# twice154/ofa-for-super-resolution

Hardware: AMD Instinct MI355X
Metric: sr_training_images_per_sec_4x_64to256 (higher is better)
Workload: dtype bf16; 1 GPU; OFA-SR S4 supernet 4x progressive shrinking (elastic kernel {3,5,7}, e=6, d=4, pd=2), LR 64x64 -> HR 256x256, fwd+bwd+Adam, train-mode BN; kernel_transform_mode=1, compat_reference_indexing=True, parallelism=dp1, per_gpu_batch=16, global_batch=16, grad_allreduce_bytes=0, launch=eager

## Files before the change

### include/ofasr.h

```cpp
#ifndef OFASR_H
#define OFASR_H

#include <stddef.h>
#include <stdint.h>

#ifdef __cplusplus
extern "C" {
#endif

#define OFASR_VERSION 312

typedef enum {
    OFASR_OK = 0,
    OFASR_ERR_INVALID_ARG = -1,
    OFASR_ERR_UNSUPPORTED = -2,
    OFASR_ERR_WORKSPACE = -3,
    OFASR_ERR_LAUNCH = -4
} ofasr_status;

typedef enum { OFASR_F32 = 0, OFASR_F16 = 1, OFASR_BF16 = 2 } ofasr_dtype;

int ofasr_version(void);
const char* ofasr_last_error_string(void);
const char* ofasr_status_string(int status);
// ... 130 lines not shown
                              void* stream);

size_t ofasr_conv2d_workspace(int64_t Cin, int64_t Cout, int K, int dgrad);
int ofasr_conv2d_stat_units(int64_t N, int64_t Cin, int64_t Cout, int64_t H, int64_t W, int K);
int ofasr_conv2d_fwd_stat(const void* x, const float* w, void* y, int64_t N, int64_t Cin, int64_t Cout, int64_t H,
                          int64_t W, int K, int dtype, void* partial, int64_t units, void* workspace,
                          size_t workspace_bytes, void* stream);
int ofasr_bn_fwd_cp(const void* x, const void* residual, void* y, const void* partial, int64_t P, const float* gamma,
                    const float* beta, float* running_mean, float* running_var, double momentum, double eps, int training,
                    float* stats, int64_t N, int64_t C, int64_t HW, int act, int dtype, void* stream);
int ofasr_bn_finalize_cp(const void* partial, int64_t P, int64_t C, double count, const float* gamma, const float* beta,
                         float* running_mean, float* running_var, double momentum, double eps, int training, float* stats,
                         void* stream);
int ofasr_pixel_shuffle2_bn(const void* x, void* y, const float* stats, int64_t N, int64_t C, int64_t H, int64_t W,
                            int dtype, void* stream);
size_t ofasr_bn_bwd_ps2_workspace(int64_t N, int64_t C);
int ofasr_bn_bwd_ps2(const void* dout, const void* x, void* dx, const float* scale, const float* mean, const float* invstd,
                     float* dgamma, float* dbeta, int64_t N, int64_t C, int64_t H, int64_t W, int training, int dtype,
                     void* workspace, size_t workspace_bytes, void* stream);
size_t ofasr_conv2d_infer_operand_bytes(int64_t Cin, int64_t Cout, int K);
int ofasr_conv2d_infer_prepare(const float* w, const float* gamma, const float* beta, const float* running_mean,
                               const float* running_var, double eps, int64_t Cin, int64_t Cout, int K, int dtype,
                               void* operands, size_t operand_bytes, void* stream);
int ofasr_conv2d_infer_run(const void* x, void* y, int64_t N, int64_t Cin, int64_t Cout, int64_t H, int64_t W, int K,
                           int dtype, int act, const void* operands, size_t operand_bytes, void* stream);
int ofasr_conv2d_fwd(const void* x, const float* w, void* y, int64_t N, int64_t Cin, int64_t Cout, int64_t H, int64_t W,
                     int K, int dtype, void* workspace, size_t workspace_bytes, void* stream);
int ofasr_conv2d_dgrad(const void* dy, const float* w, void* dx, int64_t N, int64_t Cin, int64_t Cout, int64_t H,
                       int64_t W, int K, int dtype, void* workspace, size_t workspace_bytes, void* stream);
size_t ofasr_conv2d_wgrad_workspace(int64_t N, int64_t Cin, int64_t Cout, int64_t H, int64_t W, int K);
int ofasr_conv2d_wgrad(const void* dy, const void* x, float* dw, int64_t N, int64_t Cin, int64_t Cout, int64_t H,
                       int64_t W, int K, int dtype, void* workspace, size_t workspace_bytes, void* stream);

size_t ofasr_conv2d_f32_workspace(int64_t Cin, int64_t Cout, int K, int dgrad);
// ... 117 lines not shown
```

### ofa-for-super-resolution_amd/_C.py

```python
import ctypes
import os
import subprocess

import torch

_HERE = os.path.dirname(os.path.abspath(__file__))
LIB_PATH = os.environ.get("OFASR_LIB_PATH") or os.path.join(_HERE, "csrc", "libofasr_hip.so")

F32, F16, BF16 = 0, 1, 2
U8_HWC = 3

_lib = None

_c_i64 = ctypes.c_int64
_c_int = ctypes.c_int
_c_vp = ctypes.c_void_p
_c_sz = ctypes.c_size_t

SIGNATURES = {
    "ofasr_version": (_c_int, []),
    "ofasr_last_error_string": (ctypes.c_char_p, []),
    "ofasr_status_string": (ctypes.c_char_p, [_c_int]),
    "ofasr_pixel_shuffle": (_c_int, [_c_vp, _c_vp, _c_i64, _c_i64, _c_i64, _c_i64, _c_int, _c_int, _c_vp]),
    "ofasr_pixel_unshuffle": (_c_int, [_c_vp, _c_vp, _c_i64, _c_i64, _c_i64, _c_i64, _c_int, _c_int, _c_vp]),
# ... 21 lines not shown
                                  _c_vp]),
    "ofasr_bn_fwd": (_c_int, [_c_vp, _c_vp, _c_vp, _c_vp, _c_vp, _c_vp, _c_vp, ctypes.c_double, ctypes.c_double, _c_int,
                              _c_vp, _c_i64, _c_i64, _c_i64, _c_int, _c_int, _c_vp, _c_sz, _c_vp]),
    "ofasr_bn_act_bwd_workspace": (_c_sz, [_c_i64, _c_i64]),
    "ofasr_bn_act_bwd": (_c_int, [_c_vp, _c_vp, _c_vp, _c_vp, _c_vp, _c_vp, _c_vp, _c_vp, _c_vp, _c_vp, _c_vp,
                                  _c_i64, _c_i64, _c_i64, _c_int, _c_int, _c_int, _c_vp, _c_sz, _c_vp]),
    "ofasr_conv2d_workspace": (_c_sz, [_c_i64, _c_i64, _c_int, _c_int]),
    "ofasr_conv2d_stat_units": (_c_int, [_c_i64, _c_i64, _c_i64, _c_i64, _c_i64, _c_int]),
    "ofasr_conv2d_fwd_stat": (_c_int, [_c_vp, _c_vp, _c_vp, _c_i64, _c_i64, _c_i64, _c_i64, _c_i64, _c_int, _c_int, _c_vp,
                                       _c_i64, _c_vp, _c_sz, _c_vp]),
    "ofasr_bn_fwd_cp": (_c_int, [_c_vp, _c_vp, _c_vp, _c_vp, _c_i64, _c_vp, _c_vp, _c_vp, _c_vp, ctypes.c_double,
                                 ctypes.c_double, _c_int, _c_vp, _c_i64, _c_i64, _c_i64, _c_int, _c_int, _c_vp]),
    "ofasr_bn_finalize_cp": (_c_int, [_c_vp, _c_i64, _c_i64, ctypes.c_double, _c_vp, _c_vp, _c_vp, _c_vp, ctypes.c_double,
                                      ctypes.c_double, _c_int, _c_vp, _c_vp]),
    "ofasr_pixel_shuffle2_bn": (_c_int, [_c_vp, _c_vp, _c_vp, _c_i64, _c_i64, _c_i64, _c_i64, _c_int, _c_vp]),
    "ofasr_bn_bwd_ps2_workspace": (_c_sz, [_c_i64, _c_i64]),
    "ofasr_bn_bwd_ps2": (_c_int, [_c_vp, _c_vp, _c_vp, _c_vp, _c_vp, _c_vp, _c_vp, _c_vp, _c_i64, _c_i64, _c_i64, _c_i64, _c_int,
                                  _c_int, _c_vp, _c_sz, _c_vp]),
    "ofasr_conv2d_infer_operand_bytes": (_c_sz, [_c_i64, _c_i64, _c_int]),
    "ofasr_conv2d_infer_prepare": (_c_int, [_c_vp, _c_vp, _c_vp, _c_vp, _c_vp, ctypes.c_double, _c_i64, _c_i64, _c_int, _c_int,
                                            _c_vp, _c_sz, _c_vp]),
    "ofasr_conv2d_infer_run": (_c_int, [_c_vp, _c_vp, _c_i64, _c_i64, _c_i64, _c_i64, _c_i64, _c_int, _c_int, _c_int, _c_vp,
                                        _c_sz, _c_vp]),
    "ofasr_conv2d_fwd": (_c_int, [_c_vp, _c_vp, _c_vp, _c_i64, _c_i64, _c_i64, _c_i64, _c_i64, _c_int, _c_int, _c_vp,
                                  _c_sz, _c_vp]),
    "ofasr_conv2d_dgrad": (_c_int, [_c_vp, _c_vp, _c_vp, _c_i64, _c_i64, _c_i64, _c_i64, _c_i64, _c_int, _c_int, _c_vp,
                                    _c_sz, _c_vp]),
    "ofasr_conv2d_wgrad_workspace": (_c_sz, [_c_i64, _c_i64, _c_i64, _c_i64, _c_i64, _c_int]),
    "ofasr_conv2d_wgrad": (_c_int, [_c_vp, _c_vp, _c_vp, _c_i64, _c_i64, _c_i64, _c_i64, _c_i64, _c_int, _c_int, _c_vp,
                                    _c_sz, _c_vp]),
# ... 180 lines not shown
```

### ofa-for-super-resolution_amd/csrc/conv2d.hip

```cpp
#include "ofasr_common.h"

namespace ofasr {

typedef __attribute__((ext_vector_type(16))) float cv_f32x16;
typedef __attribute__((ext_vector_type(8))) __bf16 cv_bf16x8;
typedef __attribute__((ext_vector_type(8))) _Float16 cv_f16x8;
typedef __attribute__((ext_vector_type(8))) short cv_s16x8;

constexpr int CV_TW = 64;
constexpr int CV_SEG = 20;
constexpr int CV_RP = 4 * CV_SEG;
constexpr int CV_KC = 32;

template <typename T> struct CvMma;
template <> struct CvMma<bf16_t> {
    static __device__ __forceinline__ cv_f32x16 run(cv_s16x8 a, cv_s16x8 b, cv_f32x16 c) {
        return __builtin_amdgcn_mfma_f32_32x32x16_bf16(__builtin_bit_cast(cv_bf16x8, a), __builtin_bit_cast(cv_bf16x8, b),
                                                       c, 0, 0, 0);
    }
};
template <> struct CvMma<f16_t> {
    static __device__ __forceinline__ cv_f32x16 run(cv_s16x8 a, cv_s16x8 b, cv_f32x16 c) {
        return __builtin_amdgcn_mfma_f32_32x32x16_f16(__builtin_bit_cast(cv_f16x8, a), __builtin_bit_cast(cv_f16x8, b), c,
                                                      0, 0, 0);
    }
};

__device__ __forceinline__ int cv_pos(int r, int col) { return r * CV_RP + (col & 3) * CV_SEG + (col >> 2); }
__device__ __forceinline__ int cv_rec(int P, int j) { return P * 64 + ((j ^ ((P >> 2) & 3)) << 4); }

struct CvBn {
    float* ss;
    const float* gamma;
    const float* beta;
    const float* mean;
    const float* var;
    float eps;
};

template <typename T>
__global__ void __launch_bounds__(256) conv_prep_kernel(const float* __restrict__ w, T* __restrict__ wimg, int Cin,
                                                        int KS, int dgrad, int M, int Kdim, int nrb, long long total,
                                                        CvBn bn) {
    const long long idx = (long long)blockIdx.x * blockDim.x + threadIdx.x;
    if (bn.ss != nullptr && idx < M) {
        float sc = 1.f, sh = 0.f;
        if (bn.gamma != nullptr) {
            sc = bn.gamma[idx] * rsqrtf(bn.var[idx] + bn.eps);
            sh = bn.beta[idx] - bn.mean[idx] * sc;
        }
        bn.ss[idx] = sc;
        bn.ss[M + idx] = sh;
    }
    if (idx >= total) return;
    const int j = (int)(idx & 7), lane = (int)((idx >> 3) & 63);
    long long t = idx >> 9;
    const int rb = (int)(t % nrb);
    t /= nrb;
    const int tx = (int)(t % KS);
    t /= KS;
    const int s = (int)(t & 1);
    t >>= 1;
    const int ty = (int)(t % KS);
    const int kc = (int)(t / KS);
    const int m = rb * 32 + (lane & 31), kk = kc * CV_KC + 16 * s + 8 * (lane >> 5) + j;
    float v = 0.f;
    if (m < M && kk < Kdim) {
        const int taps = KS * KS, tap = ty * KS + tx;
        v = dgrad ? w[((long long)kk * Cin + m) * taps + (taps - 1 - tap)]
                  : w[((long long)m * Cin + kk) * taps + tap];
    }
    wimg[idx] = from_float<T>(v);
}

__device__ __forceinline__ void cv_lds_barrier() { asm volatile("s_waitcnt lgkmcnt(0)\n\ts_barrier" ::: "memory"); }

struct CvEpi {
    const float* ss;
    int act;
    float2* stat;
    int P;
};

template <typename T, int KS, int RB, int WM, int WP, bool ONEK>
__global__ void __launch_bounds__(64 * WM * WP, 2) conv_igemm_kernel(const T* __restrict__ x, const T* __restrict__ wimg,
                                                                     T* __restrict__ y, int Cx, int M, int H, int W,
                                                                     int tiles_x, int nkc, int nrb, CvEpi epi) {
// ... 211 lines not shown
    p.M = (int)(dgrad ? Cin : Cout);
    p.Kdim = (int)(dgrad ? Cout : Cin);
    p.ok = (K == 3 || K == 5) && p.M > 0 && p.Kdim > 0;
    p.cfg = p.M > 128 ? 0 : (p.M > 64 ? 1 : (p.M > 32 ? 2 : 3));
    if (p.cfg == 2 && N > 0 && N * cdiv(H, 8) * cdiv(W, CV_TW) < 512) p.cfg = 4;
    p.rows = p.cfg == 0 ? 256 : (p.cfg == 1 ? 128 : (p.cfg == 3 ? 32 : 64));
    p.th = p.cfg == 0 ? 2 : ((p.cfg == 1 || p.cfg == 4) ? 4 : 8);
    p.threads = 256;
    p.nslab = (int)cdiv(p.M, p.rows);
    p.nrb = p.nslab * (p.rows / 32);
    p.nkc = (int)cdiv(p.Kdim, CV_KC);
    p.img_bytes = (size_t)p.nkc * K * 2 * K * p.nrb * 1024;
    return p;
}

template <typename T>
static int launch_conv_prep(const char* name, const float* w, int64_t Cin, int64_t Cout, int K, int dgrad, void* ws, CvBn bn,
                            hipStream_t st) {
    const CvPlan p = cv_plan(Cin, Cout, K, dgrad);
    const long long total = (long long)(p.img_bytes / 2);
    OFASR_LAUNCH((conv_prep_kernel<T>), dim3((unsigned)cdiv(total, 256)), dim3(256), 0, st, w, (T*)ws, (int)Cin, K,
                       dgrad, p.M, p.Kdim, p.nrb, total, bn);
    return check_launch(name);
}

template <typename T>
static int launch_conv_run(const char* name, const void* x, const void* ws, void* y, int64_t N, int64_t Cin, int64_t Cout,
                           int64_t H, int64_t W, int K, int dgrad, CvEpi epi, hipStream_t st) {
    const CvPlan p = cv_plan(Cin, Cout, K, dgrad, N, H, W);
    const int tiles_x = (int)cdiv(W, CV_TW), tiles_y = (int)cdiv(H, p.th);
    dim3 grid((unsigned)(tiles_x * tiles_y), (unsigned)N, (unsigned)p.nslab);
    prof_note((double)sizeof(T) * (double)N * (double)H * (double)W * (double)(Cin + Cout),
              2.0 * (double)N * (double)H * (double)W * (double)Cin * (double)Cout * K * K);
#define OFASR_CV(KS, RB, WM, WP, ONEK)                                                                                  \
    OFASR_LAUNCH((conv_igemm_kernel<T, KS, RB, WM, WP, ONEK>), grid, dim3(64 * WM * WP), 0, st, (const T*)x,         \
                       (const T*)ws, (T*)y, p.Kdim, p.M, (int)H, (int)W, tiles_x, p.nkc, p.nrb, epi)
#define OFASR_CVK(KS, ONEK)                                                                                         \
// ... 5 lines not shown
        default: OFASR_CV(KS, 1, 1, 4, ONEK); break;                                                                \
    }
    const bool onek = p.Kdim <= 16;
    if (K == 5) {
        if (onek) { OFASR_CVK(5, true) } else { OFASR_CVK(5, false) }
    } else {
        if (onek) { OFASR_CVK(3, true) } else { OFASR_CVK(3, false) }
    }
#undef OFASR_CVK
#undef OFASR_CV
    return check_launch(name);
}

template <typename T>
static int launch_conv2d(const char* name, const void* x, const float* w, void* y, int64_t N, int64_t Cin, int64_t Cout,
                         int64_t H, int64_t W, int K, int dgrad, void* ws, hipStream_t st, StatOut so = StatOut{nullptr, 0}) {
    int rc = launch_conv_prep<T>(name, w, Cin, Cout, K, dgrad, ws, CvBn{}, st);
    if (rc) return rc;
    return launch_conv_run<T>(name, x, ws, y, N, Cin, Cout, H, W, K, dgrad, CvEpi{nullptr, 0, so.partial, so.P}, st);
}

typedef __attribute__((ext_vector_type(4))) short cv_s16x4;
typedef __attribute__((address_space(3))) cv_s16x4 cv_lds_s16x4;

struct CvWgParams {
    int Cin, Cout, H, W, tiles_x, tiles_y, ntiles, ksplit, ncislab, nz;
};

template <int WCI> __device__ __forceinline__ int cvw_xoff(int R, int chunk) {
    if constexpr (WCI == 2) return R * 128 + ((((chunk >> 2) ^ ((R >> 1) & 1))) << 6) + ((chunk & 3) << 4);
    else return R * 64 + (chunk << 4);
}

// ... 264 lines not shown
    return check_launch(name);
}

static int conv_stat_units(int64_t N, int64_t Cin, int64_t Cout, int64_t H, int64_t W, int K) {
    if (conv_thin_out_supported(Cout, Cin, K, W, OFASR_BF16, nullptr, nullptr))
        return conv_thin_out_units(N, Cout, Cin, H, W, OFASR_BF16);
    if (conv_thin_in_supported(Cin, Cout, K, W, OFASR_BF16, nullptr, nullptr))
        return conv_thin_in_units(N, Cin, Cout, H, W, OFASR_BF16);
    const CvPlan p = cv_plan(Cin, Cout, K, 0, N, H, W);
    const int wp = p.th / 2;
    return (int)(N * cdiv(W, CV_TW) * cdiv(H, p.th) * wp);
}

static int conv2d_entry(const char* name, const void* x, const float* w, void* y, int64_t N, int64_t Cin, int64_t Cout,
                        int64_t H, int64_t W, int K, int dtype, int dgrad, void* ws, size_t ws_bytes, void* stream,
                        StatOut so = StatOut{nullptr, 0}) {
    OFASR_REQUIRE(x && w && y, OFASR_ERR_INVALID_ARG, "%s: null pointer", name);
    OFASR_REQUIRE(N > 0 && Cin > 0 && Cout > 0 && H > 0 && W > 0, OFASR_ERR_INVALID_ARG, "%s: bad shape", name);
    OFASR_REQUIRE(dtype == OFASR_F16 || dtype == OFASR_BF16, OFASR_ERR_UNSUPPORTED,
                  "%s: 16-bit activations only (fp32 runs on the vendor library)", name);
    OFASR_REQUIRE(K == 3 || K == 5, OFASR_ERR_UNSUPPORTED, "%s: K=%d not in {3,5}", name, K);
    OFASR_REQUIRE(W % 8 == 0 && ((reinterpret_cast<uintptr_t>(x) | reinterpret_cast<uintptr_t>(y)) & 15) == 0,
                  OFASR_ERR_UNSUPPORTED, "%s: needs W %% 8 == 0 and 16-byte aligned tensors", name);
    OFASR_REQUIRE(N <= 65535 && H * W <= (1LL << 31), OFASR_ERR_UNSUPPORTED, "%s: too large", name);
    const CvPlan p = cv_plan(Cin, Cout, K, dgrad);
    OFASR_REQUIRE(ws && ws_bytes >= p.img_bytes, OFASR_ERR_WORKSPACE, "%s: workspace %zu B < required %zu B", name,
                  ws_bytes, p.img_bytes);
    hipStream_t st = as_stream(stream);
    {
        const int64_t Ct = dgrad ? Cin : Cout, Cw = dgrad ? Cout : Cin;
        if (conv_thin_out_supported(Ct, Cw, K, W, dtype, x, y)) {
            if (so.partial)
                OFASR_REQUIRE(!dgrad && so.P == conv_thin_out_units(N, Ct, Cw, H, W, dtype), OFASR_ERR_INVALID_ARG,
                              "%s: statistics unit count %d does not match the launch", name, so.P);
            return conv_thin_out(x, w, y, N, Ct, Cw, H, W, K, dtype, dgrad, so, stream);
        }
        if (conv_thin_in_supported(Cw, Ct, K, W, dtype, x, y)) {
            if (so.partial)
                OFASR_REQUIRE(!dgrad && so.P == conv_thin_in_units(N, Cw, Ct, H, W, dtype), OFASR_ERR_INVALID_ARG,
                              "%s: statistics unit count %d does not match the launch", name, so.P);
            return conv_thin_in(x, w, y, N, Cw, Ct, H, W, K, dtype, dgrad, so, stream);
        }
    }
    if (so.partial)
        OFASR_REQUIRE(!dgrad && so.P == conv_stat_units(N, Cin, Cout, H, W, K), OFASR_ERR_INVALID_ARG,
                      "%s: statistics unit count %d does not match the launch", name, so.P);
    if (dtype == OFASR_BF16) return launch_conv2d<bf16_t>(name, x, w, y, N, Cin, Cout, H, W, K, dgrad, ws, st, so);
    return launch_conv2d<f16_t>(name, x, w, y, N, Cin, Cout, H, W, K, dgrad, ws, st, so);
}

}

using namespace ofasr;

OFASR_EXPORT size_t ofasr_conv2d_workspace(int64_t Cin, int64_t Cout, int K, int dgrad) {
    if (Cin <= 0 || Cout <= 0 || !(K == 3 || K == 5)) return 0;
    return cv_plan(Cin, Cout, K, dgrad).img_bytes;
}

OFASR_EXPORT int ofasr_conv2d_fwd(const void* x, const float* w, void* y, int64_t N, int64_t Cin, int64_t Cout, int64_t H,
                                  int64_t W, int K, int dtype, void* workspace, size_t workspace_bytes, void* stream) {
    return conv2d_entry("ofasr_conv2d_fwd", x, w, y, N, Cin, Cout, H, W, K, dtype, 0, workspace, workspace_bytes, stream);
}
// ... 53 lines not shown
                                       int64_t W, int K, int dtype, void* partial, int64_t units, void* workspace,
                                       size_t workspace_bytes, void* stream) {
    OFASR_REQUIRE(partial != nullptr && units > 0 && units <= INT32_MAX, OFASR_ERR_INVALID_ARG,
                  "ofasr_conv2d_fwd_stat: null / empty statistics buffer");
    return conv2d_entry("ofasr_conv2d_fwd_stat", x, w, y, N, Cin, Cout, H, W, K, dtype, 0, workspace, workspace_bytes, stream,
                        StatOut{(float2*)partial, (int)units});
}

OFASR_EXPORT int ofasr_conv2d_dgrad(const void* dy, const float* w, void* dx, int64_t N, int64_t Cin, int64_t Cout,
                                    int64_t H, int64_t W, int K, int dtype, void* workspace, size_t workspace_bytes,
                                    void* stream) {
    return conv2d_entry("ofasr_conv2d_dgrad", dy, w, dx, N, Cin, Cout, H, W, K, dtype, 1, workspace, workspace_bytes,
                        stream);
}

OFASR_EXPORT size_t ofasr_conv2d_wgrad_workspace(int64_t N, int64_t Cin, int64_t Cout, int64_t H, int64_t W, int K) {
    if (N <= 0 || Cin <= 0 || Cout <= 0 || H <= 0 || W <= 0 || !(K == 3 || K == 5)) return 0;
    size_t need = cv_wg_plan(N, Cin, Cout, H, W, K).part_bytes;
    const int64_t Ct = Cin < Cout ? Cin : Cout, Cw = Cin < Cout ? Cout : Cin;
    if (conv_thin_wgrad_supported(Ct, Cw, K, H, W, OFASR_BF16, nullptr, nullptr)) {
        const size_t thin = conv_thin_wgrad_workspace(N, Ct, Cw, H, W, K, OFASR_BF16);
        need = thin > need ? thin : need;
    }
    return need;
}

OFASR_EXPORT int ofasr_conv2d_wgrad(const void* dy, const void* x, float* dw, int64_t N, int64_t Cin, int64_t Cout,
                                    int64_t H, int64_t W, int K, int dtype, void* workspace, size_t workspace_bytes,
                                    void* stream) {
    const char* name = "ofasr_conv2d_wgrad";
// ... 21 lines not shown
```

### ofa-for-super-resolution_amd/csrc/pixel_shuffle.hip

```cpp
#include "ofasr_common.h"

namespace ofasr {

template <typename U, bool SHUFFLE>
__global__ void __launch_bounds__(256) ps_generic_kernel(const U* __restrict__ x, U* __restrict__ y,
                                                         int64_t total, int C, int H, int W, int r) {
    const int Ho = H * r, Wo = W * r;
    for (int64_t idx = (int64_t)blockIdx.x * blockDim.x + threadIdx.x; idx < total;
         idx += (int64_t)gridDim.x * blockDim.x) {
        int wo = (int)(idx % Wo);
        int64_t t = idx / Wo;
        int ho = (int)(t % Ho);
        t /= Ho;
        int c = (int)(t % C);
        int64_t n = t / C;
        int h = ho / r, i = ho % r, w = wo / r, j = wo % r;
        int64_t lr = (((n * C + c) * r * r + i * r + j) * H + h) * (int64_t)W + w;
        if (SHUFFLE) y[idx] = x[lr];
        else y[lr] = x[idx];
    }
}

template <int ES> struct Interleave;
template <> struct Interleave<4> {
// ... 86 lines not shown
#pragma unroll
        for (int j = 0; j < 4; ++j) {
            const float mu = mean[c0 + j], sc = scale[c0 + j];
            v[j] = ps_bn8<T>(v[j], mu, sc, fmaf(mu, sc, shift[c0 + j]));
        }
        uint4 lo, hi;
        Interleave<2>::zip(v[0], v[1], lo, hi);
        dst[hr0] = lo;
        dst[hr0 + 1] = hi;
        Interleave<2>::zip(v[2], v[3], lo, hi);
        dst[hr0 + 2 * Wq] = lo;
        dst[hr0 + 2 * Wq + 1] = hi;
    }
}

template <bool SHUFFLE>
static int launch(const void* x, void* y, int64_t N, int64_t C, int64_t H, int64_t W, int r, int es,
                  hipStream_t st) {
    const char* name = SHUFFLE ? "ofasr_pixel_shuffle" : "ofasr_pixel_unshuffle";
    OFASR_REQUIRE(x && y, OFASR_ERR_INVALID_ARG, "%s: null pointer", name);
    OFASR_REQUIRE(N >= 0 && C >= 0 && H >= 0 && W >= 0 && r >= 1, OFASR_ERR_INVALID_ARG,
                  "%s: bad shape N=%lld C=%lld H=%lld W=%lld r=%d", name, (long long)N, (long long)C,
                  (long long)H, (long long)W, r);
    OFASR_REQUIRE(es == 1 || es == 2 || es == 4 || es == 8, OFASR_ERR_UNSUPPORTED,
                  "%s: elem_size %d not in {1,2,4,8}", name, es);
    OFASR_REQUIRE(C <= INT32_MAX && H * r <= INT32_MAX && W * r <= INT32_MAX, OFASR_ERR_UNSUPPORTED,
                  "%s: dimension too large", name);
    const int64_t total = N * C * r * r * H * W;
    if (total == 0) return OFASR_OK;
    prof_note(2.0 * (double)total * es, 0.0);
// ... 53 lines not shown
    const float *mean = stats, *scale = stats + 2 * Cin, *shift = stats + 3 * Cin;
    const int Wq = (int)(W / 8);
    const int64_t items = N * C * H * Wq;
    const int64_t blocks = cdiv(items, 256);
    const int grid = (int)(blocks < 65536 ? blocks : 65536);
    hipStream_t st = as_stream(stream);
    prof_note(2.0 * 2.0 * (double)N * (double)Cin * (double)H * (double)W, 0.0);
    if (dtype == OFASR_BF16)
        OFASR_LAUNCH((ps_r2_bn_kernel<bf16_t>), dim3(grid), dim3(256), 0, st, (const uint4*)x, (uint4*)y, mean, scale, shift, items,
                     (int)C, (int)H, Wq);
    else
        OFASR_LAUNCH((ps_r2_bn_kernel<f16_t>), dim3(grid), dim3(256), 0, st, (const uint4*)x, (uint4*)y, mean, scale, shift, items,
                     (int)C, (int)H, Wq);
    return check_launch(name);
}
```

### ofa-for-super-resolution_amd/ops.py

```python
import collections
import ctypes
import os
import weakref

import torch
from torch.autograd import Function
from torch.autograd.function import once_differentiable

from . import _C

_DT = {torch.float32: _C.F32, torch.float16: _C.F16, torch.bfloat16: _C.BF16}


def _dt(t):
    try:
        return _DT[t.dtype]
    except KeyError:
        raise _C.OfasrError("unsupported activation dtype %s (f32/f16/bf16 only)" % t.dtype)


def _gpu(*ts):
    for t in ts:
        if t is None:
            continue
# ... 634 lines not shown
        if ctx.needs_input_grad[1]:
            dw = torch.zeros_like(w)
            wst, wsp, wsn = _ws(L.ofasr_pwconv_wgrad_workspace(N, Cin, cout, H * W), x.device)
            with _timed("pwconv_wgrad_%dx%d" % (cout, Cin), (x.numel() + dy.numel()) * x.element_size() + 4 * Cin * cout,
                        2 * Cin * cout * N * H * W):
                _C.check(L.ofasr_pwconv_wgrad(_p(dy), _p(x), _p(dw), ldw, N, Cin, cout, H * W, _dt(x), wsp, wsn,
                                              _stream()), "pwconv_wgrad")
        return dx, dw, None


def pwconv(x, w_full, cout):
    return PWConvFn.apply(x, w_full, cout)


ACT_NONE, ACT_RELU6 = 0, 1


class BNActFn(Function):

    @staticmethod
    def forward(ctx, x, weight, bias, running_mean, running_var, training, momentum, eps, act, residual):
        _gpu(x, weight, bias, running_mean, running_var, residual)
        x = x.contiguous()
        N, C, H, W = x.shape
        HW = H * W
        L = _C.lib()
        dev = x.device
        w = _f32_param(weight)
        b = _f32_param(bias)
        stats = torch.empty((4, C), dtype=torch.float32, device=dev)
# ... 47 lines not shown
    return dx, dgamma, dbeta, dres


class BNActCPFn(Function):

    @staticmethod
    def forward(ctx, x, partial, weight, bias, running_mean, running_var, momentum, eps, act):
        _gpu(x, weight, bias, running_mean, running_var)
        N, C, H, W = x.shape
        L = _C.lib()
        w, b = _f32_param(weight), _f32_param(bias)
        stats = torch.empty((4, C), dtype=torch.float32, device=x.device)
        units = partial.shape[1]
        if act == ACT_PIXEL_SHUFFLE2:
            y = torch.empty((N, C // 4, 2 * H, 2 * W), dtype=x.dtype, device=x.device)
            _C.check(L.ofasr_bn_finalize_cp(_p(partial), units, C, float(N * H * W), _p(w), _p(b), _p(running_mean),
                                            _p(running_var), float(momentum), float(eps), 1, _p(stats), _stream()),
                     "bn_finalize_cp")
            with _timed("bn_pixel_shuffle", 2 * x.numel() * x.element_size()):
                _C.check(L.ofasr_pixel_shuffle2_bn(_p(x), _p(y), _p(stats), N, C // 4, H, W, _dt(x), _stream()),
                         "pixel_shuffle2_bn")
        else:
            y = torch.empty_like(x)
            with _timed("bn_fwd_cp", 2 * x.numel() * x.element_size()):
                _C.check(L.ofasr_bn_fwd_cp(_p(x), None, _p(y), _p(partial), units, _p(w), _p(b), _p(running_mean),
                                           _p(running_var), float(momentum), float(eps), 1, _p(stats), N, C, H * W, int(act),
                                           _dt(x), _stream()), "bn_fwd_cp")
        ctx.save_for_backward(x, stats)
        ctx.meta = (True, ACT_NONE if act == ACT_PIXEL_SHUFFLE2 else act, False, tuple(weight.shape))
        ctx.shuffled = act == ACT_PIXEL_SHUFFLE2
        return y

    @staticmethod
    @once_differentiable
    def backward(ctx, dy):
        x, stats = ctx.saved_tensors
# ... 654 lines not shown
            return dx, None
        return dx, dw


class Conv2dFn(Function):

    @staticmethod
    def forward(ctx, x, weight, dgrad_hip=True):
        x = _al16(x.contiguous())
        N, Cin, H, W = x.shape
        Cout, _, K, _ = weight.shape
        ctx.dgrad_hip = dgrad_hip
        L = _C.lib()
        y = torch.empty((N, Cout, H, W), dtype=x.dtype, device=x.device)
        wst, wsp, wsn = _ws(L.ofasr_conv2d_workspace(Cin, Cout, K, 0), x.device)
        with _timed("conv2d_fwd_%dto%d_k%d" % (Cin, Cout, K), (x.numel() + y.numel()) * x.element_size(),
                    2 * N * H * W * Cin * Cout * K * K):
            _C.check(L.ofasr_conv2d_fwd(_p(x), _p(weight), _p(y), N, Cin, Cout, H, W, K, _dt(x), wsp, wsn, _stream()),
                     "conv2d_fwd")
        ctx.save_for_backward(x, weight)
        return y

    @staticmethod
    @once_differentiable
    def backward(ctx, dy):
        return _conv2d_backward(ctx, dy)


class Conv2dStatFn(Function):

    @staticmethod
    def forward(ctx, x, weight):
        x = _al16(x.contiguous())
        N, Cin, H, W = x.shape
        Cout, _, K, _ = weight.shape
        ctx.dgrad_hip = True
        L = _C.lib()
        y = torch.empty((N, Cout, H, W), dtype=x.dtype, device=x.device)
        units = L.ofasr_conv2d_stat_units(N, Cin, Cout, H, W, K)
        partial = torch.empty((Cout, units, 2), dtype=torch.float32, device=x.device)
        wst, wsp, wsn = _ws(L.ofasr_conv2d_workspace(Cin, Cout, K, 0), x.device)
        with _timed("conv2d_fwd_%dto%d_k%d" % (Cin, Cout, K), (x.numel() + y.numel()) * x.element_size(),
                    2 * N * H * W * Cin * Cout * K * K):
            _C.check(L.ofasr_conv2d_fwd_stat(_p(x), _p(weight), _p(y), N, Cin, Cout, H, W, K, _dt(x), _p(partial), units,
                                             wsp, wsn, _stream()), "conv2d_fwd_stat")
        ctx.save_for_backward(x, weight)
        ctx.mark_non_differentiable(partial)
        return y, partial

    @staticmethod
    @once_differentiable
    def backward(ctx, dy, _dpartial):
        return _conv2d_backward(ctx, dy)[:2]


def _conv2d_backward(ctx, dy):
    x, weight = ctx.saved_tensors
    N, Cin, H, W = x.shape
    Cout, _, K, _ = weight.shape
    dy = _al16(dy.contiguous())
    L = _C.lib()
    dx = dw = None
    if not ctx.dgrad_hip:
        w16 = weight.to(x.dtype)
        dx, dw, _ = torch.ops.aten.convolution_backward(dy, x, w16, None, [1, 1], [K // 2, K // 2], [1, 1], False,
                                                        [0, 0], 1, [ctx.needs_input_grad[0],
                                                                    ctx.needs_input_grad[1], False])
        return dx, (dw.float() if dw is not None else None), None
    cur = torch.cuda.current_stream(x.device)
    side = _side_stream(x.device) if (ctx.needs_input_grad[0] and ctx.needs_input_grad[1] and SIDE_STREAM) else None
    defer = False
    if ctx.needs_input_grad[1] and side is None and CONV_DEFER_WGRAD and H * W >= CONV_DEFER_MIN_HW \
# ... 12 lines not shown
            with torch.cuda.stream(side if side is not None else cur):
                with _timed("conv2d_wgrad_%dto%d_k%d" % (Cin, Cout, K), (x.numel() + dy.numel()) * x.element_size(),
                            2 * N * H * W * Cin * Cout * K * K):
                    _C.check(L.ofasr_conv2d_wgrad(_p(dy), _p(x), _p(dw), N, Cin, Cout, H, W, K, dt_code, wsp2, wsn2,
                                                  _stream()), "conv2d_wgrad")

        if defer and CONV_WGRAD_LATE:
            _Deferred.late.append(launch_wgrad)
        else:
            launch_wgrad()
    if ctx.needs_input_grad[0]:
        dx = torch.empty_like(x)
        wst, wsp, wsn = _ws(L.ofasr_conv2d_workspace(Cin, Cout, K, 1), x.device)
        with _timed("conv2d_dgrad_%dto%d_k%d" % (Cout, Cin, K), (x.numel() + dy.numel()) * x.element_size(),
                    2 * N * H * W * Cin * Cout * K * K):
            _C.check(L.ofasr_conv2d_dgrad(_p(dy), _p(weight), _p(dx), N, Cin, Cout, H, W, K, _dt(x), wsp, wsn,
                                          _stream()), "conv2d_dgrad")
    if defer:
        _Deferred.keep.append((x, dy, dw, wst2, weight))
        _Deferred.grads.append((weight, dw))
        _Deferred.ext_used.add(torch.device(x.device).index or 0)
        return dx, None, None
    if side is not None:
        cur.wait_stream(side)
    return dx, dw, None


ACT_PIXEL_SHUFFLE2 = 2
CONV_BN_EPILOGUE = os.environ.get("OFASR_CONV_BN_EPILOGUE", "1") != "0"
PS_BWD_FUSED = os.environ.get("OFASR_PS_BWD_FUSED", "1") != "0"


# ... 216 lines not shown
```

Measured before the change: 2807 images/s.

## Prepare dgrad weight image in forward prep kernel and fold BN finalize into pixel shuffle

The forward conv prep kernel now also writes the flipped, transposed weight image that the data-gradient conv needs, so backward can skip its own prep launch and read the saved image. Separately, the BN finalize for the pixel-shuffle path is folded into the shuffle kernel: each block reduces the per-channel partial statistics itself before normalizing. This removes two small kernel launches per affected layer. The cost is an extra saved buffer per conv held until backward, and redundant statistic reductions across blocks in the shuffle kernel.

```diff
diff --git a/include/ofasr.h b/include/ofasr.h
--- a/include/ofasr.h
+++ b/include/ofasr.h
@@ -168,10 +168,19 @@
                          void* stream);
 int ofasr_pixel_shuffle2_bn(const void* x, void* y, const float* stats, int64_t N, int64_t C, int64_t H, int64_t W,
                             int dtype, void* stream);
+int ofasr_pixel_shuffle2_bn_cp(const void* x, void* y, const void* partial, int64_t P, double count, const float* gamma,
+                               const float* beta, float* running_mean, float* running_var, double momentum, double eps,
+                               float* stats, int64_t N, int64_t C, int64_t H, int64_t W, int dtype, void* stream);
 size_t ofasr_bn_bwd_ps2_workspace(int64_t N, int64_t C);
 int ofasr_bn_bwd_ps2(const void* dout, const void* x, void* dx, const float* scale, const float* mean, const float* invstd,
                      float* dgamma, float* dbeta, int64_t N, int64_t C, int64_t H, int64_t W, int training, int dtype,
                      void* workspace, size_t workspace_bytes, void* stream);
+size_t ofasr_conv2d_dgrad_image_bytes(int64_t Cin, int64_t Cout, int64_t W, int K, int dtype);
+int ofasr_conv2d_fwd_prep2(const void* x, const float* w, void* y, int64_t N, int64_t Cin, int64_t Cout, int64_t H, int64_t W,
+                           int K, int dtype, void* partial, int64_t units, void* workspace, size_t workspace_bytes,
+                           void* dgrad_image, size_t dgrad_image_bytes, void* stream);
+int ofasr_conv2d_dgrad_prepared(const void* dy, const float* w, const void* image, size_t image_bytes, void* dx, int64_t N,
+                                int64_t Cin, int64_t Cout, int64_t H, int64_t W, int K, int dtype, void* stream);
 size_t ofasr_conv2d_infer_operand_bytes(int64_t Cin, int64_t Cout, int K);
 int ofasr_conv2d_infer_prepare(const float* w, const float* gamma, const float* beta, const float* running_mean,
                                const float* running_var, double eps, int64_t Cin, int64_t Cout, int K, int dtype,
diff --git a/ofa-for-super-resolution_amd/_C.py b/ofa-for-super-resolution_amd/_C.py
--- a/ofa-for-super-resolution_amd/_C.py
+++ b/ofa-for-super-resolution_amd/_C.py
@@ -59,6 +59,14 @@
     "ofasr_bn_finalize_cp": (_c_int, [_c_vp, _c_i64, _c_i64, ctypes.c_double, _c_vp, _c_vp, _c_vp, _c_vp, ctypes.c_double,
                                       ctypes.c_double, _c_int, _c_vp, _c_vp]),
     "ofasr_pixel_shuffle2_bn": (_c_int, [_c_vp, _c_vp, _c_vp, _c_i64, _c_i64, _c_i64, _c_i64, _c_int, _c_vp]),
+    "ofasr_pixel_shuffle2_bn_cp": (_c_int, [_c_vp, _c_vp, _c_vp, _c_i64, ctypes.c_double, _c_vp, _c_vp, _c_vp, _c_vp,
+                                            ctypes.c_double, ctypes.c_double, _c_vp, _c_i64, _c_i64, _c_i64, _c_i64, _c_int,
+                                            _c_vp]),
+    "ofasr_conv2d_dgrad_image_bytes": (_c_sz, [_c_i64, _c_i64, _c_i64, _c_int, _c_int]),
+    "ofasr_conv2d_fwd_prep2": (_c_int, [_c_vp, _c_vp, _c_vp, _c_i64, _c_i64, _c_i64, _c_i64, _c_i64, _c_int, _c_int, _c_vp,
+                                        _c_i64, _c_vp, _c_sz, _c_vp, _c_sz, _c_vp]),
+    "ofasr_conv2d_dgrad_prepared": (_c_int, [_c_vp, _c_vp, _c_vp, _c_sz, _c_vp, _c_i64, _c_i64, _c_i64, _c_i64, _c_i64,
+                                             _c_int, _c_int, _c_vp]),
     "ofasr_bn_bwd_ps2_workspace": (_c_sz, [_c_i64, _c_i64]),
     "ofasr_bn_bwd_ps2": (_c_int, [_c_vp, _c_vp, _c_vp, _c_vp, _c_vp, _c_vp, _c_vp, _c_vp, _c_i64, _c_i64, _c_i64, _c_i64, _c_int,
                                   _c_int, _c_vp, _c_sz, _c_vp]),
diff --git a/ofa-for-super-resolution_amd/csrc/conv2d.hip b/ofa-for-super-resolution_amd/csrc/conv2d.hip
--- a/ofa-for-super-resolution_amd/csrc/conv2d.hip
+++ b/ofa-for-super-resolution_amd/csrc/conv2d.hip
@@ -38,25 +38,17 @@
     float eps;
 };
 
+struct CvImg {
+    int dgrad, M, Kdim, nrb;
+    long long total;
+};
 template <typename T>
-__global__ void __launch_bounds__(256) conv_prep_kernel(const float* __restrict__ w, T* __restrict__ wimg, int Cin,
-                                                        int KS, int dgrad, int M, int Kdim, int nrb, long long total,
-                                                        CvBn bn) {
-    const long long idx = (long long)blockIdx.x * blockDim.x + threadIdx.x;
-    if (bn.ss != nullptr && idx < M) {
-        float sc = 1.f, sh = 0.f;
-        if (bn.gamma != nullptr) {
-            sc = bn.gamma[idx] * rsqrtf(bn.var[idx] + bn.eps);
-            sh = bn.beta[idx] - bn.mean[idx] * sc;
-        }
-        bn.ss[idx] = sc;
-        bn.ss[M + idx] = sh;
-    }
-    if (idx >= total) return;
+__device__ __forceinline__ void conv_prep_elem(const float* __restrict__ w, T* __restrict__ wimg, int Cin, int KS, const CvImg& g,
+                                               long long idx) {
     const int j = (int)(idx & 7), lane = (int)((idx >> 3) & 63);
     long long t = idx >> 9;
-    const int rb = (int)(t % nrb);
-    t /= nrb;
+    const int rb = (int)(t % g.nrb);
+    t /= g.nrb;
     const int tx = (int)(t % KS);
     t /= KS;
     const int s = (int)(t & 1);
@@ -65,12 +57,29 @@
     const int kc = (int)(t / KS);
     const int m = rb * 32 + (lane & 31), kk = kc * CV_KC + 16 * s + 8 * (lane >> 5) + j;
     float v = 0.f;
-    if (m < M && kk < Kdim) {
+    if (m < g.M && kk < g.Kdim) {
         const int taps = KS * KS, tap = ty * KS + tx;
-        v = dgrad ? w[((long long)kk * Cin + m) * taps + (taps - 1 - tap)]
-                  : w[((long long)m * Cin + kk) * taps + tap];
+        v = g.dgrad ? w[((long long)kk * Cin + m) * taps + (taps - 1 - tap)]
+                    : w[((long long)m * Cin + kk) * taps + tap];
     }
     wimg[idx] = from_float<T>(v);
+}
+
+template <typename T>
+__global__ void __launch_bounds__(256) conv_prep_kernel(const float* __restrict__ w, T* __restrict__ wimg, int Cin,
+                                                        int KS, CvImg a, CvBn bn, T* __restrict__ wimg_b, CvImg b) {
+    const long long idx = (long long)blockIdx.x * blockDim.x + threadIdx.x;
+    if (bn.ss != nullptr && idx < a.M) {
+        float sc = 1.f, sh = 0.f;
+        if (bn.gamma != nullptr) {
+            sc = bn.gamma[idx] * rsqrtf(bn.var[idx] + bn.eps);
+            sh = bn.beta[idx] - bn.mean[idx] * sc;
+        }
+        bn.ss[idx] = sc;
+        bn.ss[a.M + idx] = sh;
+    }
+    if (idx < a.total) conv_prep_elem<T>(w, wimg, Cin, KS, a, idx);
+    else if (idx - a.total < b.total) conv_prep_elem<T>(w, wimg_b, Cin, KS, b, idx - a.total);
 }
 
 __device__ __forceinline__ void cv_lds_barrier() { asm volatile("s_waitcnt lgkmcnt(0)\n\ts_barrier" ::: "memory"); }
@@ -312,13 +321,15 @@
     return p;
 }
 
+static CvImg cv_img(const CvPlan& p, int dgrad) { return CvImg{dgrad, p.M, p.Kdim, p.nrb, (long long)(p.img_bytes / 2)}; }
+
 template <typename T>
 static int launch_conv_prep(const char* name, const float* w, int64_t Cin, int64_t Cout, int K, int dgrad, void* ws, CvBn bn,
-                            hipStream_t st) {
-    const CvPlan p = cv_plan(Cin, Cout, K, dgrad);
-    const long long total = (long long)(p.img_bytes / 2);
-    OFASR_LAUNCH((conv_prep_kernel<T>), dim3((unsigned)cdiv(total, 256)), dim3(256), 0, st, w, (T*)ws, (int)Cin, K,
-                       dgrad, p.M, p.Kdim, p.nrb, total, bn);
+                            hipStream_t st, void* ws_b = nullptr) {
+    const CvImg a = cv_img(cv_plan(Cin, Cout, K, dgrad), dgrad);
+    const CvImg b = ws_b ? cv_img(cv_plan(Cin, Cout, K, !dgrad), !dgrad) : CvImg{0, 0, 0, 1, 0};
+    OFASR_LAUNCH((conv_prep_kernel<T>), dim3((unsigned)cdiv(a.total + b.total, 256)), dim3(256), 0, st, w, (T*)ws, (int)Cin, K,
+                       a, bn, (T*)ws_b, b);
     return check_launch(name);
 }
 
@@ -354,9 +365,12 @@
 
 template <typename T>
 static int launch_conv2d(const char* name, const void* x, const float* w, void* y, int64_t N, int64_t Cin, int64_t Cout,
-                         int64_t H, int64_t W, int K, int dgrad, void* ws, hipStream_t st, StatOut so = StatOut{nullptr, 0}) {
-    int rc = launch_conv_prep<T>(name, w, Cin, Cout, K, dgrad, ws, CvBn{}, st);
-    if (rc) return rc;
+                         int64_t H, int64_t W, int K, int dgrad, void* ws, hipStream_t st, StatOut so = StatOut{nullptr, 0},
+                         void* img_b = nullptr, bool prepared = false) {
+    if (!prepared) {
+        int rc = launch_conv_prep<T>(name, w, Cin, Cout, K, dgrad, ws, CvBn{}, st, img_b);
+        if (rc) return rc;
+    }
     return launch_conv_run<T>(name, x, ws, y, N, Cin, Cout, H, W, K, dgrad, CvEpi{nullptr, 0, so.partial, so.P}, st);
 }
 
@@ -651,7 +665,7 @@
 
 static int conv2d_entry(const char* name, const void* x, const float* w, void* y, int64_t N, int64_t Cin, int64_t Cout,
                         int64_t H, int64_t W, int K, int dtype, int dgrad, void* ws, size_t ws_bytes, void* stream,
-                        StatOut so = StatOut{nullptr, 0}) {
+                        StatOut so = StatOut{nullptr, 0}, void* img_b = nullptr, size_t img_b_bytes = 0, bool prepared = false) {
     OFASR_REQUIRE(x && w && y, OFASR_ERR_INVALID_ARG, "%s: null pointer", name);
     OFASR_REQUIRE(N > 0 && Cin > 0 && Cout > 0 && H > 0 && W > 0, OFASR_ERR_INVALID_ARG, "%s: bad shape", name);
     OFASR_REQUIRE(dtype == OFASR_F16 || dtype == OFASR_BF16, OFASR_ERR_UNSUPPORTED,
@@ -663,9 +677,16 @@
     const CvPlan p = cv_plan(Cin, Cout, K, dgrad);
     OFASR_REQUIRE(ws && ws_bytes >= p.img_bytes, OFASR_ERR_WORKSPACE, "%s: workspace %zu B < required %zu B", name,
                   ws_bytes, p.img_bytes);
+    OFASR_REQUIRE(!img_b || (img_b_bytes >= cv_plan(Cin, Cout, K, !dgrad).img_bytes && (reinterpret_cast<uintptr_t>(img_b) & 15) == 0),
+                  OFASR_ERR_WORKSPACE, "%s: second weight image %zu B < required %zu B (or not 16-byte aligned)", name, img_b_bytes,
+                  cv_plan(Cin, Cout, K, !dgrad).img_bytes);
+    OFASR_REQUIRE(!prepared || (reinterpret_cast<uintptr_t>(ws) & 15) == 0, OFASR_ERR_INVALID_ARG,
+                  "%s: a prepared weight image must be 16-byte aligned", name);
     hipStream_t st = as_stream(stream);
     {
         const int64_t Ct = dgrad ? Cin : Cout, Cw = dgrad ? Cout : Cin;
+        OFASR_REQUIRE(!img_b || !(conv_thin_out_supported(Ct, Cw, K, W, dtype, x, y) || conv_thin_in_supported(Cw, Ct, K, W, dtype, x, y)),
+                      OFASR_ERR_INVALID_ARG, "%s: the thin-side kernels read no weight image (ofasr_conv2d_dgrad_image_bytes is 0)", name);
         if (conv_thin_out_supported(Ct, Cw, K, W, dtype, x, y)) {
             if (so.partial)
                 OFASR_REQUIRE(!dgrad && so.P == conv_thin_out_units(N, Ct, Cw, H, W, dtype), OFASR_ERR_INVALID_ARG,
@@ -682,8 +703,9 @@
     if (so.partial)
         OFASR_REQUIRE(!dgrad && so.P == conv_stat_units(N, Cin, Cout, H, W, K), OFASR_ERR_INVALID_ARG,
                       "%s: statistics unit count %d does not match the launch", name, so.P);
-    if (dtype == OFASR_BF16) return launch_conv2d<bf16_t>(name, x, w, y, N, Cin, Cout, H, W, K, dgrad, ws, st, so);
-    return launch_conv2d<f16_t>(name, x, w, y, N, Cin, Cout, H, W, K, dgrad, ws, st, so);
+    if (dtype == OFASR_BF16)
+        return launch_conv2d<bf16_t>(name, x, w, y, N, Cin, Cout, H, W, K, dgrad, ws, st, so, img_b, prepared);
+    return launch_conv2d<f16_t>(name, x, w, y, N, Cin, Cout, H, W, K, dgrad, ws, st, so, img_b, prepared);
 }
 
 }
@@ -767,6 +789,30 @@
                         stream);
 }
 
+OFASR_EXPORT size_t ofasr_conv2d_dgrad_image_bytes(int64_t Cin, int64_t Cout, int64_t W, int K, int dtype) {
+    if (Cin <= 0 || Cout <= 0 || !(K == 3 || K == 5) || !(dtype == OFASR_F16 || dtype == OFASR_BF16)) return 0;
+    if (conv_thin_out_supported(Cin, Cout, K, W, dtype, nullptr, nullptr) || conv_thin_in_supported(Cout, Cin, K, W, dtype, nullptr, nullptr))
+        return 0;
+    return cv_plan(Cin, Cout, K, 1).img_bytes;
+}
+
+OFASR_EXPORT int ofasr_conv2d_fwd_prep2(const void* x, const float* w, void* y, int64_t N, int64_t Cin, int64_t Cout, int64_t H,
+                                        int64_t W, int K, int dtype, void* partial, int64_t units, void* workspace,
+                                        size_t workspace_bytes, void* dgrad_image, size_t dgrad_image_bytes, void* stream) {
+    OFASR_REQUIRE(dgrad_image != nullptr, OFASR_ERR_INVALID_ARG, "ofasr_conv2d_fwd_prep2: null image buffer");
+    OFASR_REQUIRE(partial == nullptr || (units > 0 && units <= INT32_MAX), OFASR_ERR_INVALID_ARG,
+                  "ofasr_conv2d_fwd_prep2: empty statistics buffer");
+    return conv2d_entry("ofasr_conv2d_fwd_prep2", x, w, y, N, Cin, Cout, H, W, K, dtype, 0, workspace, workspace_bytes, stream,
+                        StatOut{(float2*)partial, partial ? (int)units : 0}, dgrad_image, dgrad_image_bytes);
+}
+
+OFASR_EXPORT int ofasr_conv2d_dgrad_prepared(const void* dy, const float* w, const void* image, size_t image_bytes, void* dx,
+                                             int64_t N, int64_t Cin, int64_t Cout, int64_t H, int64_t W, int K, int dtype,
+                                             void* stream) {
+    return conv2d_entry("ofasr_conv2d_dgrad_prepared", dy, w, dx, N, Cin, Cout, H, W, K, dtype, 1, const_cast<void*>(image),
+                        image_bytes, stream, StatOut{nullptr, 0}, nullptr, 0, true);
+}
+
 OFASR_EXPORT size_t ofasr_conv2d_wgrad_workspace(int64_t N, int64_t Cin, int64_t Cout, int64_t H, int64_t W, int K) {
     if (N <= 0 || Cin <= 0 || Cout <= 0 || H <= 0 || W <= 0 || !(K == 3 || K == 5)) return 0;
     size_t need = cv_wg_plan(N, Cin, Cout, H, W, K).part_bytes;
diff --git a/ofa-for-super-resolution_amd/csrc/pixel_shuffle.hip b/ofa-for-super-resolution_amd/csrc/pixel_shuffle.hip
--- a/ofa-for-super-resolution_amd/csrc/pixel_shuffle.hip
+++ b/ofa-for-super-resolution_amd/csrc/pixel_shuffle.hip
@@ -124,6 +124,61 @@
     }
 }
 
+constexpr int PS_FOLD_ITEMS = 2048;
+template <typename T>
+__global__ void __launch_bounds__(256) ps_r2_bn_kernel_cp(const uint4* __restrict__ src, uint4* __restrict__ dst, BnFold fold,
+                                                          int Cout, int H, int Wq) {
+    __shared__ float tab[4][3];
+    const int64_t plane = (int64_t)H * Wq;
+    const int64_t nc = blockIdx.x;
+    const int c0 = 4 * (int)(nc % Cout);
+    const int64_t r0 = (int64_t)blockIdx.y * PS_FOLD_ITEMS;
+    const int64_t r1 = r0 + PS_FOLD_ITEMS < plane ? r0 + PS_FOLD_ITEMS : plane;
+    int64_t rem = r0 + threadIdx.x;
+    uint4 v[4];
+    if (rem < r1) {
+#pragma unroll
+        for (int j = 0; j < 4; ++j) v[j] = src[nc * 4 * plane + rem + j * plane];
+    }
+    {
+        const int wave = (int)(threadIdx.x >> 6), lane = (int)(threadIdx.x & 63), c = c0 + wave;
+        double s, ss;
+        bn_fold_cp_wave(fold.cp + (long long)c * fold.P, fold.P, lane, s, ss);
+        const BnMoments m = bn_moments(s, ss, fold.M);
+        const BnCoef k = bn_coef(m, fold.eps, bn_affine(fold.gamma, c, 1.0), bn_affine(fold.beta, c, 0.0));
+        if (lane == 0) {
+            const float mu = (float)m.mean;
+            tab[wave][0] = mu;
+            tab[wave][1] = k.scale;
+            tab[wave][2] = bn_beta(mu, k.scale, k.shift);
+            if (nc < Cout && blockIdx.y == 0) bn_publish(fold, c, m, k, fold.M, fold.running_mean != nullptr, false, fold.counters);
+        }
+    }
+    __syncthreads();
+    float mu[4], sc[4], be[4];
+#pragma unroll
+    for (int j = 0; j < 4; ++j) mu[j] = tab[j][0], sc[j] = tab[j][1], be[j] = tab[j][2];
+    while (rem < r1) {
+        const int h = (int)(rem / Wq);
+        const int wq = (int)(rem - (int64_t)h * Wq);
+        const int64_t hr0 = nc * 4 * plane + ((int64_t)(2 * h) * (2 * Wq)) + 2 * wq;
+#pragma unroll
+        for (int j = 0; j < 4; ++j) v[j] = ps_bn8<T>(v[j], mu[j], sc[j], be[j]);
+        uint4 lo, hi;
+        Interleave<2>::zip(v[0], v[1], lo, hi);
+        dst[hr0] = lo;
+        dst[hr0 + 1] = hi;
+        Interleave<2>::zip(v[2], v[3], lo, hi);
+        dst[hr0 + 2 * Wq] = lo;
+        dst[hr0 + 2 * Wq + 1] = hi;
+        rem += 256;
+        if (rem < r1) {
+#pragma unroll
+            for (int j = 0; j < 4; ++j) v[j] = src[nc * 4 * plane + rem + j * plane];
+        }
+    }
+}
+
 template <bool SHUFFLE>
 static int launch(const void* x, void* y, int64_t N, int64_t C, int64_t H, int64_t W, int r, int es,
                   hipStream_t st) {
@@ -207,3 +262,33 @@
                      (int)C, (int)H, Wq);
     return check_launch(name);
 }
+
+OFASR_EXPORT int ofasr_pixel_shuffle2_bn_cp(const void* x, void* y, const void* partial, int64_t P, double count, const float* gamma,
+                                            const float* beta, float* running_mean, float* running_var, double momentum,
+                                            double eps, float* stats, int64_t N, int64_t C, int64_t H, int64_t W, int dtype,
+                                            void* stream) {
+    using namespace ofasr;
+    const char* name = "ofasr_pixel_shuffle2_bn_cp";
+    OFASR_REQUIRE(x && y && stats && partial, OFASR_ERR_INVALID_ARG, "%s: null pointer", name);
+    OFASR_REQUIRE(N > 0 && C > 0 && H > 0 && W > 0 && P > 0 && P <= INT32_MAX && count > 0, OFASR_ERR_INVALID_ARG, "%s: bad shape", name);
+    OFASR_REQUIRE((running_mean == nullptr) == (running_var == nullptr), OFASR_ERR_INVALID_ARG, "%s: half a pair of running statistics", name);
+    OFASR_REQUIRE(dtype == OFASR_F16 || dtype == OFASR_BF16, OFASR_ERR_UNSUPPORTED, "%s: 16-bit tensors only", name);
+    OFASR_REQUIRE(W % 8 == 0 && ((reinterpret_cast<uintptr_t>(x) | reinterpret_cast<uintptr_t>(y)) & 15) == 0,
+                  OFASR_ERR_UNSUPPORTED, "%s: needs W %% 8 == 0 and 16-byte aligned tensors", name);
+    OFASR_REQUIRE(C <= INT32_MAX / 4 && 2 * H <= INT32_MAX && 2 * W <= INT32_MAX && N * C <= INT32_MAX, OFASR_ERR_UNSUPPORTED,
+                  "%s: too large", name);
+    const int64_t Cin = 4 * C;
+    const int Wq = (int)(W / 8);
+    const int64_t chunks = cdiv(H * Wq, (int64_t)PS_FOLD_ITEMS);
+    OFASR_REQUIRE(chunks <= 65535, OFASR_ERR_UNSUPPORTED, "%s: plane too large", name);
+    const BnFold fold{(const float2*)partial, (int)P, count, momentum, eps, gamma, beta, running_mean, running_var,
+                      stats, stats + Cin, stats + 2 * Cin, stats + 3 * Cin, {nullptr, nullptr, nullptr}};
+    const dim3 grid((unsigned)(N * C), (unsigned)chunks);
+    hipStream_t st = as_stream(stream);
+    prof_note(2.0 * 2.0 * (double)N * (double)Cin * (double)H * (double)W, 0.0);
+    if (dtype == OFASR_BF16)
+        OFASR_LAUNCH((ps_r2_bn_kernel_cp<bf16_t>), grid, dim3(256), 0, st, (const uint4*)x, (uint4*)y, fold, (int)C, (int)H, Wq);
+    else
+        OFASR_LAUNCH((ps_r2_bn_kernel_cp<f16_t>), grid, dim3(256), 0, st, (const uint4*)x, (uint4*)y, fold, (int)C, (int)H, Wq);
+    return check_launch(name);
+}
diff --git a/ofa-for-super-resolution_amd/ops.py b/ofa-for-super-resolution_amd/ops.py
--- a/ofa-for-super-resolution_amd/ops.py
+++ b/ofa-for-super-resolution_amd/ops.py
@@ -672,6 +672,7 @@
 
 
 ACT_NONE, ACT_RELU6 = 0, 1
+PS_BN_FOLD = os.environ.get("OFASR_PS_BN_FOLD", "1") != "0"
 
 
 class BNActFn(Function):
@@ -749,12 +750,19 @@
         units = partial.shape[1]
         if act == ACT_PIXEL_SHUFFLE2:
             y = torch.empty((N, C // 4, 2 * H, 2 * W), dtype=x.dtype, device=x.device)
-            _C.check(L.ofasr_bn_finalize_cp(_p(partial), units, C, float(N * H * W), _p(w), _p(b), _p(running_mean),
-                                            _p(running_var), float(momentum), float(eps), 1, _p(stats), _stream()),
-                     "bn_finalize_cp")
-            with _timed("bn_pixel_shuffle", 2 * x.numel() * x.element_size()):
-                _C.check(L.ofasr_pixel_shuffle2_bn(_p(x), _p(y), _p(stats), N, C // 4, H, W, _dt(x), _stream()),
-                         "pixel_shuffle2_bn")
+            if PS_BN_FOLD:
+                with _timed("bn_pixel_shuffle", 2 * x.numel() * x.element_size()):
+                    _C.check(L.ofasr_pixel_shuffle2_bn_cp(_p(x), _p(y), _p(partial), units, float(N * H * W), _p(w), _p(b),
+                                                          _p(running_mean), _p(running_var), float(momentum), float(eps),
+                                                          _p(stats), N, C // 4, H, W, _dt(x), _stream()),
+                             "pixel_shuffle2_bn_cp")
+            else:
+                _C.check(L.ofasr_bn_finalize_cp(_p(partial), units, C, float(N * H * W), _p(w), _p(b), _p(running_mean),
+                                                _p(running_var), float(momentum), float(eps), 1, _p(stats), _stream()),
+                         "bn_finalize_cp")
+                with _timed("bn_pixel_shuffle", 2 * x.numel() * x.element_size()):
+                    _C.check(L.ofasr_pixel_shuffle2_bn(_p(x), _p(y), _p(stats), N, C // 4, H, W, _dt(x), _stream()),
+                             "pixel_shuffle2_bn")
         else:
             y = torch.empty_like(x)
             with _timed("bn_fwd_cp", 2 * x.numel() * x.element_size()):
@@ -1439,11 +1447,16 @@
         L = _C.lib()
         y = torch.empty((N, Cout, H, W), dtype=x.dtype, device=x.device)
         wst, wsp, wsn = _ws(L.ofasr_conv2d_workspace(Cin, Cout, K, 0), x.device)
+        dimg = _dgrad_image(ctx, x, weight) if dgrad_hip else None
         with _timed("conv2d_fwd_%dto%d_k%d" % (Cin, Cout, K), (x.numel() + y.numel()) * x.element_size(),
                     2 * N * H * W * Cin * Cout * K * K):
-            _C.check(L.ofasr_conv2d_fwd(_p(x), _p(weight), _p(y), N, Cin, Cout, H, W, K, _dt(x), wsp, wsn, _stream()),
-                     "conv2d_fwd")
-        ctx.save_for_backward(x, weight)
+            if dimg is not None:
+                _C.check(L.ofasr_conv2d_fwd_prep2(_p(x), _p(weight), _p(y), N, Cin, Cout, H, W, K, _dt(x), None, 0, wsp, wsn,
+                                                  _p(dimg), dimg.numel(), _stream()), "conv2d_fwd_prep2")
+            else:
+                _C.check(L.ofasr_conv2d_fwd(_p(x), _p(weight), _p(y), N, Cin, Cout, H, W, K, _dt(x), wsp, wsn, _stream()),
+                         "conv2d_fwd")
+        ctx.save_for_backward(x, weight, dimg)
         return y
 
     @staticmethod
@@ -1465,22 +1478,45 @@
         units = L.ofasr_conv2d_stat_units(N, Cin, Cout, H, W, K)
         partial = torch.empty((Cout, units, 2), dtype=torch.float32, device=x.device)
         wst, wsp, wsn = _ws(L.ofasr_conv2d_workspace(Cin, Cout, K, 0), x.device)
+        dimg = _dgrad_image(ctx, x, weight)
         with _timed("conv2d_fwd_%dto%d_k%d" % (Cin, Cout, K), (x.numel() + y.numel()) * x.element_size(),
                     2 * N * H * W * Cin * Cout * K * K):
-            _C.check(L.ofasr_conv2d_fwd_stat(_p(x), _p(weight), _p(y), N, Cin, Cout, H, W, K, _dt(x), _p(partial), units,
-                                             wsp, wsn, _stream()), "conv2d_fwd_stat")
-        ctx.save_for_backward(x, weight)
+            if dimg is not None:
+                _C.check(L.ofasr_conv2d_fwd_prep2(_p(x), _p(weight), _p(y), N, Cin, Cout, H, W, K, _dt(x), _p(partial), units,
+                                                  wsp, wsn, _p(dimg), dimg.numel(), _stream()), "conv2d_fwd_prep2")
+            else:
+                _C.check(L.ofasr_conv2d_fwd_stat(_p(x), _p(weight), _p(y), N, Cin, Cout, H, W, K, _dt(x), _p(partial), units,
+                                                 wsp, wsn, _stream()), "conv2d_fwd_stat")
+        ctx.save_for_backward(x, weight, dimg)
         ctx.mark_non_differentiable(partial)
+        ctx.set_materialize_grads(False)
         return y, partial
 
     @staticmethod
     @once_differentiable
     def backward(ctx, dy, _dpartial):
+        if dy is None:
+            return None, None
         return _conv2d_backward(ctx, dy)[:2]
 
 
+CONV_PREP_ONCE = os.environ.get("OFASR_CONV_PREP_ONCE", "1") != "0"
+DGRAD_IMAGES = [0]
+
+
+def _dgrad_image(ctx, x, weight):
+    if not (CONV_PREP_ONCE and ctx.needs_input_grad[0]):
+        return None
+    Cout, Cin, K, _ = weight.shape
+    n = _C.lib().ofasr_conv2d_dgrad_image_bytes(Cin, Cout, x.shape[3], K, _dt(x))
+    if n == 0:
+        return None
+    DGRAD_IMAGES[0] += 1
+    return torch.empty(n, dtype=torch.uint8, device=x.device)
+
+
 def _conv2d_backward(ctx, dy):
-    x, weight = ctx.saved_tensors
+    x, weight, dimg = ctx.saved_tensors
     N, Cin, H, W = x.shape
     Cout, _, K, _ = weight.shape
     dy = _al16(dy.contiguous())
@@ -1523,8 +1559,12 @@
         wst, wsp, wsn = _ws(L.ofasr_conv2d_workspace(Cin, Cout, K, 1), x.device)
         with _timed("conv2d_dgrad_%dto%d_k%d" % (Cout, Cin, K), (x.numel() + dy.numel()) * x.element_size(),
                     2 * N * H * W * Cin * Cout * K * K):
-            _C.check(L.ofasr_conv2d_dgrad(_p(dy), _p(weight), _p(dx), N, Cin, Cout, H, W, K, _dt(x), wsp, wsn,
-                                          _stream()), "conv2d_dgrad")
+            if dimg is not None:
+                _C.check(L.ofasr_conv2d_dgrad_prepared(_p(dy), _p(weight), _p(dimg), dimg.numel(), _p(dx), N, Cin, Cout, H, W,
+                                                       K, _dt(x), _stream()), "conv2d_dgrad_prepared")
+            else:
+                _C.check(L.ofasr_conv2d_dgrad(_p(dy), _p(weight), _p(dx), N, Cin, Cout, H, W, K, _dt(x), wsp, wsn,
+                                              _stream()), "conv2d_dgrad")
     if defer:
         _Deferred.keep.append((x, dy, dw, wst2, weight))
         _Deferred.grads.append((weight, dw))
```

Result: no change. 2817 images/s, median of 6 (+0.4%).
